# szy4017/DeepSense6G_TII

Hardware: AMD Instinct MI355X
Metric: training samples/sec (5-frame seq, bs=12 per GPU) (higher is better)
Workload: dtype f32; 1 GPU; BASELINE configs[2]: full camera+LiDAR+radar+GPS fusion, 5x(3+1+2)x256x256 + 2x2 GPS per sample, bs=12 per GPU, sigmoid focal loss, AdamW, train-mode BN, dropout 0.1; global_batch=12, seq_len=5, parallelism=dp1, ema=False, launch=eager, optimizer=AdamW after backward

## Files before the change

### deepsense6g_tii_amd/csrc/attention.hip

```cpp
#include "common.h"

int g_ds6g_attn_percu = 0;
int g_ds6g_attn_handover = 1;
int g_ds6g_attn_merged_sum = 1;
thread_local int g_attn_bwd_slab_sums = 0;
int g_ds6g_attn_fused128 = 1;

#ifdef DS6G_ATTN_CLOCKS
__device__ unsigned long long g_attn_clk[16];
extern "C" int ds6g_attn_clocks_read(unsigned long long* out16, int reset) {
    if (hipMemcpyFromSymbol(out16, HIP_SYMBOL(g_attn_clk), sizeof(unsigned long long) * 16) != hipSuccess) return -1;
    if (reset) {
        unsigned long long z[16] = {};
        if (hipMemcpyToSymbol(HIP_SYMBOL(g_attn_clk), z, sizeof(z)) != hipSuccess) return -1;
    }
    return 0;
}
#define ATTN_CLK_DECL() unsigned long long clk_t_ = 0; const bool clk_on_ = blockIdx.x == 0 && blockIdx.y == 0 && blockIdx.z == 0 && threadIdx.x == 0;
#define ATTN_CLK_START() do { __builtin_amdgcn_sched_barrier(0); clk_t_ = __builtin_readcyclecounter(); } while (0)
#define ATTN_CLK(ph) do { __builtin_amdgcn_sched_barrier(0); const unsigned long long n_ = __builtin_readcyclecounter(); \
        if (clk_on_) g_attn_clk[ph] += n_ - clk_t_; clk_t_ = n_; } while (0)
#else
#define ATTN_CLK_DECL()
#define ATTN_CLK_START()
#define ATTN_CLK(ph)
#endif

namespace {

struct AttnParams {
    const float* q;
    const float* k;
    const float* v;
    float* o;
    float* lse;
    float* ml;
    const float* d_o;
    float* delta;
    float* dq;
    float* dk;
    float* dv;
    int T, nh, B;
    int ld;
    int ldq;
    int ldd;
    int splits, tiles_per_split;
    size_t slab;
    unsigned bytes;
    unsigned bytes_q;
    float scale;
    uint32_t thr;
    float dscale;
    uint64_t seed;
    uint64_t seed_off;
    const uint64_t* salt;
    float* hs;
    float* hp;
    int nkg;
    int out16;
// ... 778 lines not shown
                ds_out[g * 64] = key_ok ? f32x4{dp[4 * g], dp[4 * g + 1], dp[4 * g + 2], dp[4 * g + 3]} : f32x4{0.f, 0.f, 0.f, 0.f};
            }
            if (PART == 2) {
                f32x4* p_out = reinterpret_cast<f32x4*>(p.hp + tile);
#pragma unroll
                for (int g = 0; g < 4; ++g)
                    p_out[g * 64] = key_ok ? f32x4{s[4 * g], s[4 * g + 1], s[4 * g + 2], s[4 * g + 3]} : f32x4{0.f, 0.f, 0.f, 0.f};
            }
        }
        __builtin_amdgcn_sched_barrier(0);
        ATTN_CLK(4);
        if (DO_DV) mma_dims<HD, BF>(dv, Oc, s, dtab);
        __builtin_amdgcn_sched_barrier(0);
        ATTN_CLK(5);
        if (DO_DK) mma_dims<HD, BF>(dk, Qc, dp, dtab);
        __builtin_amdgcn_sched_barrier(0);
        ATTN_CLK(6);
        if (HAND) asm volatile("s_waitcnt vmcnt(%0)" ::"n"((BF >= 4 ? 2 : 4) + (PART == 2 ? 4 : 0)) : "memory");
        else asm volatile("s_waitcnt vmcnt(0)" ::: "memory");
        ATTN_CLK(7);
        __syncthreads();
        ATTN_CLK(8);
#ifdef DS6G_ATTN_CLOCKS
        if (clk_on_) g_attn_clk[15] += 1;
#endif
    };

    if (t_begin < t_end) {
        q_ld.issue(Xa0, t_begin * 32, wave);
        do_ld.issue(Xb0, t_begin * 32, wave);
        stats(t_begin, 0);
    }
    asm volatile("s_waitcnt vmcnt(0)" ::: "memory");
    __syncthreads();
    for (int qt = t_begin; qt < t_end; qt += 2) {
        step(Xa0, Xb0, Xa1, Xb1, qt, 0, qt + 1 < t_end);
        if (qt + 1 < t_end) step(Xa1, Xb1, Xa0, Xb0, qt + 1, 1, qt + 2 < t_end);
    }
    if (p.splits == 1 && p.out16) {
        if (DO_DK) store_rows16<HD, BF>(dk, reinterpret_cast<typename AttnT16<BF>::T*>(p.dk) + head_offd, p.ldd, key, T, half, 1.0f);
        if (DO_DV) store_rows16<HD, BF>(dv, reinterpret_cast<typename AttnT16<BF>::T*>(p.dv) + head_offd, p.ldd, key, T, half, 1.0f);
    } else if (p.splits == 1) {
        if (DO_DK) store_rows<HD, BF>(dk, p.dk + head_offd, p.ldd, key, T, half, 1.0f);
        if (DO_DV) store_rows<HD, BF>(dv, p.dv + head_offd, p.ldd, key, T, half, 1.0f);
    } else {
        if (DO_DK) store_rows<HD, BF>(dk, p.dk + (size_t)split * p.slab + head_off, p.ld, key, T, half, 1.0f);
        if (DO_DV) store_rows<HD, BF>(dv, p.dv + (size_t)split * p.slab + head_off, p.ld, key, T, half, 1.0f);
    }
}

__global__ __launch_bounds__(256) void attn_delta_kernel(const float* __restrict__ o, const float* __restrict__ d_o,
                                                         float* __restrict__ delta, int B, int T, int nh, int hd, int ld,
                                                         int o16) {
    const long i = (long)blockIdx.x * blockDim.x + threadIdx.x;
    if (i >= (long)B * T * nh) return;
    const int h = (int)(i % nh);
    const long row = i / nh;
    const float* a = o + row * ld + h * hd;
    const float* g = d_o + row * ld + h * hd;
    float acc = 0.f;
    if (o16 == 6) {
        const _Float16* a16 = reinterpret_cast<const _Float16*>(o) + row * ld + h * hd;
        const _Float16* g16 = reinterpret_cast<const _Float16*>(d_o) + row * ld + h * hd;
        for (int d = 0; d < hd; d += 4) {
            const f32x4 x = ld4(a16 + d), y = ld4(g16 + d);
            acc += x[0] * y[0] + x[1] * y[1] + x[2] * y[2] + x[3] * y[3];
        }
    } else if (o16 == 3) {
        typedef __bf16 bf16x4_ __attribute__((ext_vector_type(4)));
        const __bf16* a16 = reinterpret_cast<const __bf16*>(o) + row * ld + h * hd;
        const __bf16* g16 = reinterpret_cast<const __bf16*>(d_o) + row * ld + h * hd;
        for (int d = 0; d < hd; d += 4) {
            const bf16x4_ x = *reinterpret_cast<const bf16x4_*>(a16 + d), y = *reinterpret_cast<const bf16x4_*>(g16 + d);
            acc += (float)x[0] * (float)y[0] + (float)x[1] * (float)y[1] + (float)x[2] * (float)y[2] + (float)x[3] * (float)y[3];
        }
    } else if (o16) {
        typedef __bf16 bf16x4_ __attribute__((ext_vector_type(4)));
        const __bf16* a16 = reinterpret_cast<const __bf16*>(o) + row * ld + h * hd;
        for (int d = 0; d < hd; d += 4) {
            const bf16x4_ x = *reinterpret_cast<const bf16x4_*>(a16 + d);
            const f32x4 y = *reinterpret_cast<const f32x4*>(g + d);
            acc += (float)x[0] * y[0] + (float)x[1] * y[1] + (float)x[2] * y[2] + (float)x[3] * y[3];
        }
    } else
    for (int d = 0; d < hd; d += 4) {
        const f32x4 x = *reinterpret_cast<const f32x4*>(a + d), y = *reinterpret_cast<const f32x4*>(g + d);
        acc += x[0] * y[0] + x[1] * y[1] + x[2] * y[2] + x[3] * y[3];
    }
    const int b = (int)(row / T), t = (int)(row % T);
    delta[((long)b * nh + h) * T + t] = acc;
}

template <int HD, int BF>
__global__ __launch_bounds__(256, 2) void attn_bwd_dq2_kernel(const AttnParams p) {
    __shared__ __attribute__((aligned(16))) float Xa0[32 * HD];
    __shared__ __attribute__((aligned(16))) float Xa1[32 * HD];
    __shared__ float Tr[4][32 * 33];
    ATTN_GEOM();
    const int q_row = bx_ * 128 + wave * 32 + l31;
    const int qt = bx_ * 4 + wave;
    const TileLoader<HD, BF> k_ld(p.k, (long)b * T * p.ldq, T, p.ldq, h * HD, wave, lane);
    f32x16 dq[NB];
#pragma unroll
    for (int blk = 0; blk < NB; ++blk)
#pragma unroll
        for (int r = 0; r < 16; ++r) dq[blk][r] = 0.f;
    const float* tiles = p.hs + (((size_t)(b * p.nh + h) * p.nkg + qt) * p.nkg) * 1024 + lane * 4;
    const bool have = qt < ntiles;
    float f[16], fn[16];
    auto fetch = [&](float* dst, int kt) {
        if (BF >= 4) {
            typedef typename AttnT16<BF>::T T16;
            typedef typename H16<T16>::x8 h8;
            const T16* t16 = reinterpret_cast<const T16*>(p.hs) + ((((size_t)(b * p.nh + h) * p.nkg + qt) * p.nkg) + kt) * 1024 + lane * 8;
#pragma unroll
            for (int g = 0; g < 2; ++g) {
                h8 v;
                if (have) v = *reinterpret_cast<const h8*>(t16 + g * 512);
#pragma unroll
                for (int e = 0; e < 8; ++e) dst[8 * g + e] = have ? (float)v[e] : 0.f;
            }
            return;
        }
#pragma unroll
        for (int g = 0; g < 4; ++g) {
            const f32x4 v = have ? *reinterpret_cast<const f32x4*>(tiles + (size_t)kt * 1024 + g * 256) : f32x4{0.f, 0.f, 0.f, 0.f};
            dst[4 * g] = v[0]; dst[4 * g + 1] = v[1]; dst[4 * g + 2] = v[2]; dst[4 * g + 3] = v[3];
        }
    };
    float* tw = Tr[wave];
    auto step = [&](const float* Kcp, const float* Kn, int kt, bool more) {
        if (more) {
            k_ld.issue(Kn, (kt + 1) * 32, wave);
            fetch(fn, kt + 1);
        }
        const unsigned Kc = opaque_tile(Kcp);
#pragma unroll
        for (int r = 0; r < 16; ++r) tw[krow16(r, half) * 33 + l31] = f[r];
        __builtin_amdgcn_wave_barrier();
        f32x16 s;
#pragma unroll
        for (int r = 0; r < 16; ++r) s[r] = tw[l31 * 33 + krow16(r, half)];
        __builtin_amdgcn_wave_barrier();
// ... 263 lines not shown
}

AttnParams attn_params(const float* q, const float* k, const float* v, int in16, float* lse, int out16, int B, int T, int nh, int hd,
                       int ld_qkv, int ld, int ld_out, float drop_p, uint64_t seed, uint64_t seed_off) {
    AttnParams p{};
    p.q = q; p.k = k; p.v = v; p.lse = lse; p.T = T; p.nh = nh; p.B = B; p.ld = ld; p.ldq = ld_qkv; p.ldd = ld_out;
    p.in16 = in16; p.out16 = out16;
    const size_t esz = in16 ? 2 : 4;
    p.slab = (size_t)B * T * ld; p.bytes = (unsigned)(p.slab * esz);
    p.bytes_q = (unsigned)((((size_t)B * T - 1) * ld_qkv + nh * hd) * esz);
    p.scale = 1.0f / sqrtf((float)hd);
    ds6g_attn_drop_params(drop_p, &p.thr, &p.dscale); p.seed = seed; p.seed_off = seed_off; p.salt = g_ds6g_salt;
    p.nkg = cdiv(T, 128) * 4;
    return p;
}

int attention_run(bool backward, const AttnParams& c, int hd, void* ws, size_t ws_bytes, void* stream) {
    const AttnKnobs kn = attn_knobs();
    const AttnShape s(c.in16 ? DS6G_ATTN_KIND_H16 : (c.out16 ? DS6G_ATTN_KIND_OUT16 : DS6G_ATTN_KIND_F32), c.B, c.T, c.nh, hd, c.ld);
    ds6g_attn_plan plan;
    int rc = DS6G_OK;
    if (backward) rc = plan_bwd(s, ws ? ws_bytes : 0, kn, &plan);
    else plan_fwd(s, ws ? ws_bytes : 0, kn, &plan);
    DS6G_CHECK_WS(rc != DS6G_ERR_WORKSPACE);
    DS6G_CHECK_ARG(rc == DS6G_OK);
    if (backward) g_attn_bwd_slab_sums = plan.slab_sums;

    static float* AttnParams::* const field[DS6G_ATTN_T_COUNT] = {&AttnParams::o, &AttnParams::ml, &AttnParams::dq, &AttnParams::dk,
                                                                   &AttnParams::dv, &AttnParams::delta, &AttnParams::hs, &AttnParams::hp};
    hipStream_t st = (hipStream_t)stream;
    AttnParams p = c;
    const int bf = c.in16 ? 3 + c.in16 : kn.bf16;
    const int cols4 = c.nh * hd / 4;
    const long n4 = (long)c.B * c.T * cols4;
    for (int i = 0; i < plan.nsteps; ++i) {
        const ds6g_attn_step& step = plan.steps[i];
        const ds6g_attn_out* o = step.out;
        float *at[3] = {}, *mine[3] = {};
        for (int j = 0; j < step.nout; ++j) { at[j] = (float*)((char*)ws + o[j].off); mine[j] = c.*field[o[j].tensor]; }
        if (step.splits) {
            p.splits = step.splits; p.tiles_per_split = step.tiles_per_split;
            for (int j = 0; j < step.nout; ++j) p.*field[o[j].tensor] = o[j].slabs ? at[j] : mine[j];
        }
        const dim3 grid(cdiv(c.T, 128), c.nh * step.splits, c.B);
        switch (step.family) {
            case DS6G_ATTN_FWD: rc = launch<DS6G_ATTN_FWD>(bf, p, hd, grid, st); break;
            case DS6G_ATTN_DQ_RECOMPUTE: rc = launch<DS6G_ATTN_DQ_RECOMPUTE>(bf, p, hd, grid, st); break;
            case DS6G_ATTN_DKV_RECOMPUTE: rc = launch<DS6G_ATTN_DKV_RECOMPUTE>(bf, p, hd, grid, st); break;
            case DS6G_ATTN_DKV_HANDOVER: rc = launch<DS6G_ATTN_DKV_HANDOVER>(bf, p, hd, grid, st); break;
            case DS6G_ATTN_DKV_FUSED128: rc = launch<DS6G_ATTN_DKV_FUSED128>(bf, p, hd, grid, st); break;
            case DS6G_ATTN_DK_TWO_PASS: rc = launch<DS6G_ATTN_DK_TWO_PASS>(bf, p, hd, grid, st); break;
            case DS6G_ATTN_DV_FROM_P: rc = launch<DS6G_ATTN_DV_FROM_P>(bf, p, hd, grid, st); break;
            case DS6G_ATTN_DQ_FROM_DS: rc = launch<DS6G_ATTN_DQ_FROM_DS>(bf, p, hd, grid, st); break;
            case DS6G_ATTN_DELTA:
                hipLaunchKernelGGL(attn_delta_kernel, dim3(cdiv((long)c.B * c.T * c.nh, 256)), dim3(256), 0, st, c.o, c.d_o, c.delta,
                                   c.B, c.T, c.nh, hd, c.ld, c.o16 | (c.in16 << 1));
                break;
            case DS6G_ATTN_FWD_MERGE:
                hipLaunchKernelGGL(attn_fwd_merge_kernel, dim3(cdiv(n4, 256)), dim3(256), 0, st, at[0], at[1], c.o, c.lse, c.B, c.T,
                                   c.nh, hd, c.ld, o[0].slabs, c.slab, c.out16);
                break;
            case DS6G_ATTN_SLAB_SUM:
                hipLaunchKernelGGL(slab_sum_kernel, dim3(cdiv(n4, 256), step.nout), dim3(256), 0, st, at[0], mine[0], at[1], mine[1],
                                   n4, cols4, c.ld, c.ldd, o[0].slabs, c.slab, c.out16, at[2], mine[2], o[2].slabs);
                break;
        }
        if (rc) return rc;
        DS6G_LAUNCH_CHECK();
    }
    return DS6G_OK;
}

}

extern "C" {

size_t ds6g_attention_workspace_bytes(int B, int T, int nh, int hd, int ld) {
    return AttnShape(DS6G_ATTN_KIND_F32, B, T, nh, hd, ld).full_workspace();
}

int ds6g_attention_plan(int backward, int kind, int B, int T, int nh, int hd, int ld, size_t ws_bytes, ds6g_attn_plan* plan) {
    DS6G_CHECK_ARG(plan && kind >= DS6G_ATTN_KIND_F32 && kind <= DS6G_ATTN_KIND_H16 && B > 0 && T > 0 && nh > 0);
    DS6G_CHECK_ARG((hd == 16 || hd == 32 || hd == 64 || hd == 128) && ld % 4 == 0 && ld >= nh * hd);
    DS6G_CHECK_ARG((size_t)B * T * ld * sizeof(float) < OOB_OFF);
    const AttnShape s(kind, B, T, nh, hd, ld);
    if (backward) return plan_bwd(s, ws_bytes, attn_knobs(), plan);
    plan_fwd(s, ws_bytes, attn_knobs(), plan);
    return DS6G_OK;
}

static int attention_fwd_impl(const float* q, const float* k, const float* v, int in16, float* o, int out16, float* lse, int B, int T,
                              int nh, int hd, int ld_qkv, int ld, float drop_p, uint64_t seed, uint64_t seed_off, void* ws,
                              size_t ws_bytes, void* stream) {
    DS6G_ENTER();
    DS6G_CHECK_ARG(q && k && v && o && lse && B > 0 && T > 0 && ld % 4 == 0 && ld >= nh * hd);
    DS6G_CHECK_ARG(ld_qkv % 4 == 0 && ld_qkv >= nh * hd && (size_t)B * T * ld_qkv * sizeof(float) < OOB_OFF);
    DS6G_CHECK_ARG(drop_p >= 0.f && drop_p < 1.f);
    DS6G_CHECK_ARG((size_t)B * T * ld * sizeof(float) < OOB_OFF);
    AttnParams c = attn_params(q, k, v, in16, lse, out16, B, T, nh, hd, ld_qkv, ld, ld, drop_p, seed, seed_off);
    c.o = o;
    return attention_run(false, c, hd, ws, ws_bytes, stream);
}

int ds6g_attention_fwd(const float* q, const float* k, const float* v, float* o, float* lse, int B, int T, int nh,
                       int hd, int ld_qkv, int ld, float drop_p, uint64_t seed, uint64_t seed_off, void* ws,
                       size_t ws_bytes, void* stream) {
    return attention_fwd_impl(q, k, v, 0, o, 0, lse, B, T, nh, hd, ld_qkv, ld, drop_p, seed, seed_off, ws, ws_bytes, stream);
}
int ds6g_attention_fwd_bf16out(const float* q, const float* k, const float* v, void* o, float* lse, int B, int T, int nh,
                               int hd, int ld_qkv, int ld, float drop_p, uint64_t seed, uint64_t seed_off, void* ws,
// ... 57 lines not shown
```

### deepsense6g_tii_amd/csrc/igemm.hip

```cpp
#include "common.h"
#include "gemm_plan.h"
#include <type_traits>
#include <vector>

extern int g_ds6g_attn_fused128;
extern int g_ds6g_attn_merged_sum;
extern int g_ds6g_attn_percu;
extern int g_ds6g_attn_handover;
extern int g_wino_kb64;

#ifndef IGEMM_STAGES_FD
#define IGEMM_STAGES_FD 3
#endif
#ifndef IGEMM_STAGES_W
#define IGEMM_STAGES_W 2
#endif

GCLK_STORAGE(g_igemm_clk, g_igemm_wg, ds6g_igemm_clocks_read)

namespace {

enum { MODE_FWD = 0, MODE_DGRAD = 1, MODE_WGRAD = 2 };

__device__ __forceinline__ unsigned opaque_u32(unsigned x) {
    asm volatile("" : "+v"(x));
    return x;
}

struct IgemmParams {
    const float* a_src;
    const float* b_src;
    float* out;
    int N, H, W, C;
    int Ho, Wo, K;
    int R, S, stride, pad;
    int Mg, Ng, Kg;
    const float* bias;
    const float* residual;
    const float* mask_src;
    int relu;
    int accumulate;
    uint32_t drop_thr;
    float drop_scale;
    uint64_t seed;
    uint64_t seed_off;
    const uint64_t* salt;
    int k_per_split;
    size_t split_stride;
    int tiles_n;
    int nclass;
    double prof_flops;
    int wg_rows;
    int is_linear;
    int want_colsum;
    int xcd_splits;
    int h0, hstep, Hs, w0, wstep, Ws, r0, rstep, nr, s0, sstep, ns;
    unsigned a_bytes, b_bytes;
    int dbg;
};


// ... 789 lines not shown
                           dim3(256), 0, st, p);
}

int run_igemm(const IgemmParams& p, const GemmPlan& pl, float* dw, float* dbias, int accumulate, hipStream_t st) {
    void* rec = ds6g_prof_open(pl.variant, p.prof_flops > 0 ? p.prof_flops : 2.0 * p.Mg * p.Ng * p.Kg, st);
    const int code = ((pl.tile * 2 + pl.epilogue) * 3 + (pl.bk == 32 ? 2 : pl.walk)) * 4 + pl.operand_mode;
    const auto codes = std::make_integer_sequence<int, 3 * 2 * 3 * 4>{};
    if (pl.mode == MODE_FWD) gemm_dispatch(code, [&](auto c) { launch_igemm<MODE_FWD, decltype(c)::value>(p, pl, st); }, codes);
    else if (pl.mode == MODE_DGRAD) gemm_dispatch(code, [&](auto c) { launch_igemm<MODE_DGRAD, decltype(c)::value>(p, pl, st); }, codes);
    else gemm_dispatch(code, [&](auto c) { launch_igemm<MODE_WGRAD, decltype(c)::value>(p, pl, st); }, codes);
    ds6g_prof_close(rec, st);
    g_last_variant = pl.variant;
    DS6G_LAUNCH_CHECK();
    if (!pl.reduce) return DS6G_OK;
    return ds6g_internal_splitk_reduce(p.out, dw, (long)pl.Mg * pl.Ng / 4, dbias, pl.want_colsum ? pl.Mg / 4 : 0, pl.splits,
                                       pl.slab_elems, accumulate, accumulate, st);
}

constexpr int F32 = DS6G_GEMM_F32;

}

extern "C" {

int ds6g_last_igemm_variant(void) { return g_last_variant; }

int ds6g_profile_begin(int max_records) {
    if (max_records <= 0) return DS6G_ERR_ARG;
    if (!g_prof) g_prof = new std::vector<ProfRec>();
    for (auto& r : *g_prof) { (void)hipEventDestroy(r.e0); (void)hipEventDestroy(r.e1); }
    g_prof->clear();
    g_prof->reserve((size_t)max_records);
    g_prof_cap = (size_t)max_records;
    return DS6G_OK;
}

int ds6g_profile_end(int* variants, double* flops, float* ms, int cap) {
    if (!g_prof) return 0;
    int n = 0;
    for (auto& r : *g_prof) {
        (void)hipEventSynchronize(r.e1);
        float t = 0.f;
        (void)hipEventElapsedTime(&t, r.e0, r.e1);
        if (n < cap && variants && flops && ms) { variants[n] = r.variant; flops[n] = r.flops; ms[n] = t; ++n; }
        (void)hipEventDestroy(r.e0);
        (void)hipEventDestroy(r.e1);
    }
    g_prof->clear();
    g_prof_cap = 0;
    return n;
}

int ds6g_set_debug_flags(int flags) {
    g_knobs.dbg = flags & 0xbf;
    g_ds6g_attn_handover = (flags & 0x01000000) ? 0 : 1;
    g_ds6g_attn_fused128 = (flags & 0x04000000) ? 0 : 1;
    g_ds6g_attn_merged_sum = (flags & 0x08000000) ? 0 : 1;
    g_ds6g_attn_percu = (flags >> 20) & 0xf;
    g_wino_kb64 = (flags & 0x02000000) ? 1 : 0;
    g_knobs.bf16_bk32 = (flags & 0x10000000) ? 0 : 1;
    g_knobs.f32_bk32 = (flags & 0x20000000) ? 1 : ((flags & 0x40000000) ? 0 : 2);
    g_knobs.wgrad_tile = (flags & 0x40) ? 2 : 1;
    if ((flags >> 8) & 0xfff) g_knobs.min_blocks = (flags >> 8) & 0xfff;
    return 0;
}

int ds6g_gemm_plan(int family, int op, int N, int H, int W, int C, int K, int R, int S, int stride, int pad, int flags,
                   size_t ws_bytes, struct ds6g_gemm_plan* plan) {
    const GemmProblem q = {family, op, N, H, W, C, K, R, S, stride, pad, (flags & DS6G_GEMM_EPILOGUE) != 0,
                           (flags & DS6G_GEMM_OUT16) != 0, (flags & DS6G_GEMM_ACCUMULATE) != 0, (flags & DS6G_GEMM_DBIAS) != 0, ws_bytes};
    return gemm_plan(q, family == DS6G_GEMM_H16 ? ds6g_internal_bgemm_knobs() : igemm_knobs(), plan);
}

int ds6g_conv2d_fwd(const float* x, const float* w, float* y, int N, int H, int W, int C, int K, int R,
                    int S, int stride, int pad, void* stream) {
    DS6G_ENTER();
    DS6G_CHECK_ARG(x && w && y);
    const GemmProblem q = {F32, DS6G_GEMM_CONV_FWD, N, H, W, C, K, R, S, stride, pad, 0, 0, 0, 0, 0};
    GemmPlan pl; IgemmParams p;
    if (const int rc = plan_params(q, pl, p)) return rc;
    p.a_src = x; p.b_src = w; p.out = y;
    return run_igemm(p, pl, nullptr, nullptr, 0, (hipStream_t)stream);
}

int ds6g_conv2d_dgrad(const float* dy, const float* w, float* dx, int N, int H, int W, int C, int K, int R,
                      int S, int stride, int pad, int accumulate, void* stream) {
    DS6G_ENTER();
    DS6G_CHECK_ARG(dy && w && dx);
    const GemmProblem q = {F32, DS6G_GEMM_CONV_DGRAD, N, H, W, C, K, R, S, stride, pad, 0, 0, accumulate, 0, 0};
    GemmPlan pl; IgemmParams p;
    if (const int rc = plan_params(q, pl, p)) return rc;
    p.a_src = dy; p.b_src = w; p.out = dx;
    return run_igemm(p, pl, nullptr, nullptr, 0, (hipStream_t)stream);
}

int ds6g_conv2d_wgrad(const float* x, const float* dy, float* dw, int N, int H, int W, int C, int K, int R,
                      int S, int stride, int pad, int accumulate, float* ws, size_t ws_bytes, void* stream) {
    DS6G_ENTER();
    DS6G_CHECK_ARG(x && dy && dw);
    const GemmProblem q = {F32, DS6G_GEMM_CONV_WGRAD, N, H, W, C, K, R, S, stride, pad, 0, 0, accumulate, 0, ws_bytes};
    GemmPlan pl; IgemmParams p;
    if (const int rc = plan_params(q, pl, p)) return rc;
    DS6G_CHECK_ARG(ws || !pl.reduce);
    p.a_src = dy; p.b_src = x; p.out = pl.reduce ? ws : dw;
    return run_igemm(p, pl, dw, nullptr, accumulate, (hipStream_t)stream);
}
// ... 53 lines not shown
```

### deepsense6g_tii_amd/csrc/norm.hip

```cpp
#include "common.h"

namespace {

constexpr int BN_ROWS_PER_THREAD = 16;
constexpr int BNF_COLS = 2;
constexpr int BNF_GROUPS = 128;

__device__ __forceinline__ void bnf_reduce2(double& a, double& b, double (*red)[4][BNF_COLS]) {
#pragma unroll
    for (int o = BNF_COLS; o < 64; o <<= 1) {
        a += __shfl_xor(a, o, 64);
        b += __shfl_xor(b, o, 64);
    }
    const int lane = threadIdx.x & 63, wave = threadIdx.x >> 6;
    if (lane < BNF_COLS) {
        red[0][wave][lane] = a;
        red[1][wave][lane] = b;
    }
    __syncthreads();
    if (threadIdx.x < BNF_COLS) {
        a = red[0][0][threadIdx.x] + red[0][1][threadIdx.x] + red[0][2][threadIdx.x] + red[0][3][threadIdx.x];
        b = red[1][0][threadIdx.x] + red[1][1][threadIdx.x] + red[1][2][threadIdx.x] + red[1][3][threadIdx.x];
    }
}

template <int MODE, typename TX, typename TA>
__global__ __launch_bounds__(256) void bn_reduce_kernel(const TX* __restrict__ x, const TA* __restrict__ dy,
                                                        const TA* __restrict__ y_mask,
                                                        const float* __restrict__ mean,
                                                        const float* __restrict__ invstd, long M, int C,
                                                        int rows_per_block, double* __restrict__ partial,
                                                        const float* __restrict__ mg, const float* __restrict__ mb,
                                                        const PoolGrad pg) {
    extern __shared__ __attribute__((aligned(16))) double red[];
    const int cg = C >> 2;
    const int colg = threadIdx.x % cg;
    const int rowlane = threadIdx.x / cg;
    const int rowlanes = 256 / cg;
    const long r0 = (long)blockIdx.x * rows_per_block;
    const long r1 = min(M, r0 + rows_per_block);
    f32x4 s1 = {0.f, 0.f, 0.f, 0.f}, s2 = {0.f, 0.f, 0.f, 0.f};
    f32x4 mu = {0.f, 0.f, 0.f, 0.f}, is = {1.f, 1.f, 1.f, 1.f};
    f32x4 gam = {1.f, 1.f, 1.f, 1.f}, bet = {0.f, 0.f, 0.f, 0.f};
    if (MODE == 1) {
        mu = *reinterpret_cast<const f32x4*>(mean + colg * 4);
        is = *reinterpret_cast<const f32x4*>(invstd + colg * 4);
        if (mg) {
            gam = *reinterpret_cast<const f32x4*>(mg + colg * 4);
            bet = *reinterpret_cast<const f32x4*>(mb + colg * 4);
        }
    }
    for (long r = r0 + rowlane; r < r1; r += rowlanes) {
        const size_t o = (size_t)r * C + colg * 4;
        const f32x4 xv = ld4(x + o);
        if (MODE == 0) {
            s1 += xv;
            s2 += xv * xv;
        } else {
            f32x4 g = pg.dp ? pooled_grad(pg, r, colg * 4, C) : ld4(dy + o);
            if (y_mask || mg) {
                const f32x4 yv = mg ? bn_affine(xv, mu, is, gam, bet) : ld4(y_mask + o);
#pragma unroll
                for (int j = 0; j < 4; ++j) g[j] = yv[j] > 0.f ? g[j] : 0.f;
            }
            s1 += g;
            s2 += g * ((xv - mu) * is);
        }
    }
    double* mine = red + ((size_t)rowlane * 2) * C + colg * 4;
#pragma unroll
    for (int j = 0; j < 4; ++j) {
        mine[j] = (double)s1[j];
        mine[C + j] = (double)s2[j];
    }
    __syncthreads();
    for (int i = threadIdx.x; i < 2 * C; i += 256) {
        double acc = 0.0;
        for (int rl = 0; rl < rowlanes; ++rl) acc += red[(size_t)rl * 2 * C + i];
        partial[(size_t)blockIdx.x * 2 * C + i] = acc;
    }
}

__global__ __launch_bounds__(256) void bn_stats_finalize_kernel(const double* __restrict__ partial, int nblk, long M,
                                                                int C, float eps, float momentum,
                                                                float* __restrict__ mean, float* __restrict__ invstd,
                                                                float* __restrict__ running_mean,
                                                                float* __restrict__ running_var) {
    __shared__ double red[2][4][BNF_COLS];
    const int cl = threadIdx.x & (BNF_COLS - 1), g = threadIdx.x / BNF_COLS;
    const int c = blockIdx.x * BNF_COLS + cl;
    double s = 0.0, q = 0.0;
    if (c < C)
        for (int b = g; b < nblk; b += BNF_GROUPS) {
            s += partial[(size_t)b * 2 * C + c];
            q += partial[(size_t)b * 2 * C + C + c];
        }
    bnf_reduce2(s, q, red);
    if (g != 0 || c >= C) return;
    const double mu = s / (double)M;
    double var = q / (double)M - mu * mu;
    if (var < 0.0) var = 0.0;
    mean[c] = (float)mu;
    invstd[c] = (float)(1.0 / sqrt(var + (double)eps));
    if (running_mean) {
        const double unbiased = M > 1 ? var * ((double)M / (double)(M - 1)) : var;
        running_mean[c] = (float)((1.0 - momentum) * (double)running_mean[c] + momentum * mu);
        running_var[c] = (float)((1.0 - momentum) * (double)running_var[c] + momentum * unbiased);
    }
}

__global__ void bn_eval_prepare_kernel(const float* __restrict__ running_mean, const float* __restrict__ running_var,
                                       int C, float eps, float* __restrict__ mean, float* __restrict__ invstd) {
    const int c = blockIdx.x * blockDim.x + threadIdx.x;
    if (c >= C) return;
    mean[c] = running_mean[c];
    invstd[c] = 1.0f / sqrtf(running_var[c] + eps);
// ... 11 lines not shown
        const int c4 = (int)(i % cg) * 4;
        const f32x4 mu = *reinterpret_cast<const f32x4*>(mean + c4);
        const f32x4 is = *reinterpret_cast<const f32x4*>(invstd + c4);
        const f32x4 g = *reinterpret_cast<const f32x4*>(gamma + c4);
        const f32x4 b = *reinterpret_cast<const f32x4*>(beta + c4);
        f32x4 v = ld4(x + i * 4);
        v = bn_affine(v, mu, is, g, b);
        if (residual) v += ld4(residual + i * 4);
        if (relu) {
#pragma unroll
            for (int j = 0; j < 4; ++j) v[j] = fmaxf(v[j], 0.f);
        }
        st4(y + i * 4, v);
    }
}

__global__ __launch_bounds__(256) void bn_bwd_finalize_kernel(const double* __restrict__ partial, int nblk, long M,
                                                              int C, const float* __restrict__ gamma,
                                                              const float* __restrict__ invstd,
                                                              float* __restrict__ dgamma, float* __restrict__ dbeta,
                                                              float* __restrict__ coef, int accumulate) {
    __shared__ double red[2][4][BNF_COLS];
    const int cl = threadIdx.x & (BNF_COLS - 1), g = threadIdx.x / BNF_COLS;
    const int c = blockIdx.x * BNF_COLS + cl;
    double s1 = 0.0, s2 = 0.0;
    if (c < C)
        for (int b = g; b < nblk; b += BNF_GROUPS) {
            s1 += partial[(size_t)b * 2 * C + c];
            s2 += partial[(size_t)b * 2 * C + C + c];
        }
    bnf_reduce2(s1, s2, red);
    if (g != 0 || c >= C) return;
    if (accumulate) {
        dgamma[c] += (float)s2;
        dbeta[c] += (float)s1;
    } else {
        dgamma[c] = (float)s2;
        dbeta[c] = (float)s1;
    }
    coef[c] = gamma[c] * invstd[c];
    coef[C + c] = (float)(s1 / (double)M);
    coef[2 * C + c] = (float)(s2 / (double)M);
}

template <typename TX, typename TA>
__global__ __launch_bounds__(256) void bn_bwd_apply_kernel(const TA* __restrict__ dy,
                                                           const TA* __restrict__ y_mask,
                                                           const TX* __restrict__ x,
                                                           const float* __restrict__ mean,
                                                           const float* __restrict__ invstd,
                                                           const float* __restrict__ coef, TX* __restrict__ dx,
                                                           TA* __restrict__ dres, long total4, int C,
                                                           const float* __restrict__ mg, const float* __restrict__ mb,
                                                           const PoolGrad pg) {
    const int cg = C >> 2;
    for (long i = (long)blockIdx.x * blockDim.x + threadIdx.x; i < total4; i += (long)gridDim.x * blockDim.x) {
        const int c4 = (int)(i % cg) * 4;
        const f32x4 mu = *reinterpret_cast<const f32x4*>(mean + c4);
        const f32x4 is = *reinterpret_cast<const f32x4*>(invstd + c4);
        const f32x4 a = *reinterpret_cast<const f32x4*>(coef + c4);
        const f32x4 b = *reinterpret_cast<const f32x4*>(coef + C + c4);
        const f32x4 cc = *reinterpret_cast<const f32x4*>(coef + 2 * C + c4);
        f32x4 g = pg.dp ? pooled_grad(pg, i / cg, c4, C) : ld4(dy + i * 4);
        const f32x4 xv = ld4(x + i * 4);
        if (y_mask || mg) {
            const f32x4 yv = mg ? bn_affine(xv, mu, is, *reinterpret_cast<const f32x4*>(mg + c4),
                                            *reinterpret_cast<const f32x4*>(mb + c4))
                                : ld4(y_mask + i * 4);
#pragma unroll
            for (int j = 0; j < 4; ++j) g[j] = yv[j] > 0.f ? g[j] : 0.f;
        }
        const f32x4 xh = (xv - mu) * is;
        if (dres) st4(dres + i * 4, g);
        st4(dx + i * 4, a * (g - b - xh * cc));
    }
}

int bn_geometry(long M, int C, int* rows_per_block, int* nblk) {
    const int cg = C / 4;
    if (C % 4 != 0 || cg > 256 || 256 % cg != 0) return DS6G_ERR_ARG;
    *rows_per_block = BN_ROWS_PER_THREAD * (256 / cg);
    *nblk = cdiv(M, *rows_per_block);
    return DS6G_OK;
}

template <int C>
struct LnRow {
    static constexpr bool VEC = C >= 256;
    static constexpr int NV = VEC ? C / 256 : C / 64;
    static constexpr int NE = VEC ? 4 * NV : NV;
    __device__ static void load(float* v, const float* row, int lane) {
        if (VEC) {
#pragma unroll
            for (int j = 0; j < NV; ++j) {
                const f32x4 t = *reinterpret_cast<const f32x4*>(row + 4 * lane + 256 * j);
                v[4 * j] = t[0]; v[4 * j + 1] = t[1]; v[4 * j + 2] = t[2]; v[4 * j + 3] = t[3];
            }
        } else {
#pragma unroll
            for (int j = 0; j < NV; ++j) v[j] = row[lane + 64 * j];
        }
    }
    __device__ static void store(const float* v, float* row, int lane) {
        if (VEC) {
#pragma unroll
            for (int j = 0; j < NV; ++j)
                *reinterpret_cast<f32x4*>(row + 4 * lane + 256 * j) = f32x4{v[4 * j], v[4 * j + 1], v[4 * j + 2], v[4 * j + 3]};
        } else {
#pragma unroll
            for (int j = 0; j < NV; ++j) row[lane + 64 * j] = v[j];
        }
    }
    __device__ static int col(int e, int lane) { return VEC ? 4 * lane + 256 * (e >> 2) + (e & 3) : lane + 64 * e; }
    template <typename T16>
    __device__ static void load(float* v, const T16* row, int lane) {
        typedef typename H16<T16>::x4 h4;
        if (VEC) {
#pragma unroll
            for (int j = 0; j < NV; ++j) {
                const h4 t = *reinterpret_cast<const h4*>(row + 4 * lane + 256 * j);
                v[4 * j] = (float)t[0]; v[4 * j + 1] = (float)t[1]; v[4 * j + 2] = (float)t[2]; v[4 * j + 3] = (float)t[3];
            }
        } else {
#pragma unroll
            for (int j = 0; j < NV; ++j) v[j] = (float)row[lane + 64 * j];
        }
// ... 168 lines not shown
    const int rowlanes = 256 / cols_per_pass;
    const int rowlane = threadIdx.x / cols_per_pass;
    const long r0 = (long)blockIdx.x * rows_per_block;
    const long r1 = min(M, r0 + rows_per_block);
    for (int cbase = 0; cbase < cg; cbase += cols_per_pass) {
        const int colg = cbase + threadIdx.x % cols_per_pass;
        f32x4 s = {0.f, 0.f, 0.f, 0.f};
        if (colg < cg)
            for (long r = r0 + rowlane; r < r1; r += rowlanes) s += *reinterpret_cast<const f32x4*>(x + (size_t)r * C + colg * 4);
        if (colg < cg) *reinterpret_cast<f32x4*>(redf + (size_t)rowlane * C + colg * 4) = s;
    }
    __syncthreads();
    for (int c = threadIdx.x; c < C; c += 256) {
        float acc = 0.f;
        for (int rl = 0; rl < rowlanes; ++rl) acc += redf[(size_t)rl * C + c];
        partial[(size_t)blockIdx.x * C + c] = acc;
    }
}

template <typename TW>
__global__ __launch_bounds__(256) void bn_fold_kernel(const float* __restrict__ w, const float* __restrict__ gamma,
                                                      const float* __restrict__ beta, const float* __restrict__ mean,
                                                      const float* __restrict__ var, float eps, TW* __restrict__ w_out,
                                                      float* __restrict__ bias_out, int K, int taps, int cin, int cpad) {
    const long i = (long)blockIdx.x * blockDim.x + threadIdx.x;
    const long per_o = (long)taps * cpad;
    if (i >= (long)K * per_o) return;
    const int o = (int)(i / per_o);
    const int rem = (int)(i - (long)o * per_o);
    const int tap = rem / cpad, c = rem - tap * cpad;
    const float scale = gamma[o] / sqrtf(var[o] + eps);
    float v = c < cin ? w[((long)o * taps + tap) * cin + c] * scale : 0.f;
    if constexpr (sizeof(TW) == 2) asm volatile("" : "+v"(v));
    w_out[i] = (TW)v;
    if (rem == 0) bias_out[o] = beta[o] - mean[o] * scale;
}

}

extern "C" size_t ds6g_layernorm_bwd_workspace_bytes(int M, int C);
extern "C" size_t ds6g_bn_workspace_bytes(long M, int C);

template <typename TX>
static int bn_stats_run(const TX* x, long M, int C, float eps, float momentum, float* mean, float* invstd,
                        float* running_mean, float* running_var, void* ws, size_t ws_bytes, void* stream) {
    int rpb, nblk;
    DS6G_CHECK_ARG(x && mean && invstd && ws && M > 0);
    DS6G_CHECK_ARG(bn_geometry(M, C, &rpb, &nblk) == DS6G_OK);
    DS6G_CHECK_WS(ws_bytes >= ds6g_bn_workspace_bytes(M, C));
    double* partial = (double*)ws;
    const size_t lds = (size_t)(256 / (C / 4)) * 2 * C * sizeof(double);
    hipLaunchKernelGGL((bn_reduce_kernel<0, TX, TX>), dim3(nblk), dim3(256), lds, (hipStream_t)stream, x, (const TX*)nullptr,
                       (const TX*)nullptr, (const float*)nullptr, (const float*)nullptr, M, C, rpb, partial,
                       (const float*)nullptr, (const float*)nullptr, PoolGrad{});
    DS6G_LAUNCH_CHECK();
    hipLaunchKernelGGL(bn_stats_finalize_kernel, dim3(cdiv(C, BNF_COLS)), dim3(256), 0, (hipStream_t)stream, partial, nblk,
                       M, C, eps, momentum, mean, invstd, running_mean, running_var);
    DS6G_LAUNCH_CHECK();
    return DS6G_OK;
}

template <typename TA>
static int bn_apply_run(const TA* x, const float* mean, const float* invstd, const float* gamma, const float* beta,
                        const TA* residual, TA* y, long M, int C, int relu, void* stream) {
    DS6G_CHECK_ARG(x && mean && invstd && gamma && beta && y && C % 4 == 0);
    const long total4 = M * C / 4;
    const int grid = (int)min((long)8192, (total4 + 255) / 256);
    hipLaunchKernelGGL((bn_apply_kernel<TA>), dim3(grid), dim3(256), 0, (hipStream_t)stream, x, mean, invstd, gamma, beta,
                       residual, y, total4, C, relu);
    DS6G_LAUNCH_CHECK();
    return DS6G_OK;
}

template <typename TX, typename TA>
static int bn_bwd_run(const TA* dy, const PoolGrad pg, const TA* y_mask, const TX* x, const float* mean,
                      const float* invstd, const float* gamma, const float* relu_beta, TX* dx, float* dgamma,
                      float* dbeta, TA* dres, long M, int C, int accumulate_param_grads, void* ws, size_t ws_bytes,
                      void* stream) {
    const float* mg = relu_beta ? gamma : nullptr;
    int rpb, nblk;
    DS6G_CHECK_ARG(bn_geometry(M, C, &rpb, &nblk) == DS6G_OK);
    DS6G_CHECK_WS(ws_bytes >= ds6g_bn_workspace_bytes(M, C));
    double* partial = (double*)ws;
    float* coef = (float*)((char*)ws + (size_t)nblk * 2 * C * sizeof(double));
    const size_t lds = (size_t)(256 / (C / 4)) * 2 * C * sizeof(double);
    hipLaunchKernelGGL((bn_reduce_kernel<1, TX, TA>), dim3(nblk), dim3(256), lds, (hipStream_t)stream, x, dy, y_mask, mean,
                       invstd, M, C, rpb, partial, mg, relu_beta, pg);
    DS6G_LAUNCH_CHECK();
    hipLaunchKernelGGL(bn_bwd_finalize_kernel, dim3(cdiv(C, BNF_COLS)), dim3(256), 0, (hipStream_t)stream, partial, nblk, M,
                       C, gamma, invstd, dgamma, dbeta, coef, accumulate_param_grads);
    DS6G_LAUNCH_CHECK();
    const long total4 = M * C / 4;
    const int grid = (int)min((long)8192, (total4 + 255) / 256);
    hipLaunchKernelGGL((bn_bwd_apply_kernel<TX, TA>), dim3(grid), dim3(256), 0, (hipStream_t)stream, dy, y_mask, x, mean,
                       invstd, coef, dx, dres, total4, C, mg, relu_beta, pg);
    DS6G_LAUNCH_CHECK();
    return DS6G_OK;
}

template <typename TY>
static int ln_fwd_launch(const float* x, const float* gamma, const float* beta, TY* y, float* mean, float* rstd, int M, int C,
                         float eps, hipStream_t st) {
    dim3 grid(cdiv(M, 4)), block(256);
    switch (C / 64) {
        case 1: hipLaunchKernelGGL((ln_fwd_kernel<64, TY>), grid, block, 0, st, x, gamma, beta, y, mean, rstd, M, eps); break;
        case 2: hipLaunchKernelGGL((ln_fwd_kernel<128, TY>), grid, block, 0, st, x, gamma, beta, y, mean, rstd, M, eps); break;
        case 4: hipLaunchKernelGGL((ln_fwd_kernel<256, TY>), grid, block, 0, st, x, gamma, beta, y, mean, rstd, M, eps); break;
        case 8: hipLaunchKernelGGL((ln_fwd_kernel<512, TY>), grid, block, 0, st, x, gamma, beta, y, mean, rstd, M, eps); break;
        default: DS6G_CHECK_ARG(!"LayerNorm width must be 64/128/256/512");
    }
    DS6G_LAUNCH_CHECK();
    return DS6G_OK;
}

template <typename TDY, typename TDD>
static int ln_bwd_launch(const TDY* dy, const float* x, const float* mean, const float* rstd, const float* gamma,
                         const float* add, float* dx, float* dgamma, float* dbeta, int M, int C, int accumulate_param_grads,
                         TDD* dx_drop, float drop_p, uint64_t seed, uint64_t seed_off, void* ws, size_t ws_bytes,
                         hipStream_t st, bool defer = false) {
    DS6G_CHECK_ARG(dy && x && mean && rstd && gamma && dx && (defer || (dgamma && dbeta)) && ws && M > 0);
    DS6G_CHECK_ARG(drop_p >= 0.f && drop_p < 1.f);
    const uint32_t thr = ds6g_drop_threshold(drop_p);
    const float dscale = 1.f / (1.f - drop_p);
    DS6G_CHECK_ARG(C % 64 == 0 && C <= 512);
    DS6G_CHECK_WS(ws_bytes >= ds6g_layernorm_bwd_workspace_bytes(M, C));
    const int nblk = cdiv(M, LN_BWD_ROWS);
    float* partial = (float*)ws;
    dim3 grid(nblk), block(256);
    switch (C / 64) {
        case 1: hipLaunchKernelGGL((ln_bwd_kernel<64, TDY, TDD>), grid, block, 0, st, dy, x, mean, rstd, gamma, add, dx, partial, M, dx_drop, thr, dscale, seed, seed_off, g_ds6g_salt); break;
        case 2: hipLaunchKernelGGL((ln_bwd_kernel<128, TDY, TDD>), grid, block, 0, st, dy, x, mean, rstd, gamma, add, dx, partial, M, dx_drop, thr, dscale, seed, seed_off, g_ds6g_salt); break;
        case 4: hipLaunchKernelGGL((ln_bwd_kernel<256, TDY, TDD>), grid, block, 0, st, dy, x, mean, rstd, gamma, add, dx, partial, M, dx_drop, thr, dscale, seed, seed_off, g_ds6g_salt); break;
        case 8: hipLaunchKernelGGL((ln_bwd_kernel<512, TDY, TDD>), grid, block, 0, st, dy, x, mean, rstd, gamma, add, dx, partial, M, dx_drop, thr, dscale, seed, seed_off, g_ds6g_salt); break;
        default: DS6G_CHECK_ARG(!"LayerNorm width must be 64/128/256/512");
    }
    DS6G_LAUNCH_CHECK();
    if (defer) return DS6G_OK;
    hipLaunchKernelGGL(col_finalize_kernel, dim3(cdiv(2 * C, 4)), dim3(256), 0, st, partial, nblk, 2 * C, dgamma,
                       dbeta, C, accumulate_param_grads);
    DS6G_LAUNCH_CHECK();
    return DS6G_OK;
}

int ds6g_internal_bn_stats_finalize(const double* partial, int nblk, long M, int C, float eps, float momentum, float* mean,
                                    float* invstd, float* running_mean, float* running_var, hipStream_t st) {
    hipLaunchKernelGGL(bn_stats_finalize_kernel, dim3(cdiv(C, BNF_COLS)), dim3(256), 0, st, partial, nblk, M, C, eps,
                       momentum, mean, invstd, running_mean, running_var);
    DS6G_LAUNCH_CHECK();
// ... 280 lines not shown
```

Before: 187.7 samples/s.

## Coalesce attention delta reduction and reuse masked BN grad from reduce pass

Adds a streaming attention-delta kernel in which threads load contiguous quads of o and dO, with coalesced accesses, and write partial dot products to LDS. A second loop sums each head's terms, replacing the one-thread-per-row strided loop. Separately, the BN backward reduce pass now stores the ReLU-masked gradient into dres, so the apply pass reads it back instead of re-reading dy and y_mask. Both paths are on by default with debug flags to revert, and fp contraction is disabled so the delta arithmetic stays consistent between the two kernels.

```diff
diff --git a/deepsense6g_tii_amd/csrc/attention.hip b/deepsense6g_tii_amd/csrc/attention.hip
--- a/deepsense6g_tii_amd/csrc/attention.hip
+++ b/deepsense6g_tii_amd/csrc/attention.hip
@@ -5,6 +5,7 @@
 int g_ds6g_attn_merged_sum = 1;
 thread_local int g_attn_bwd_slab_sums = 0;
 int g_ds6g_attn_fused128 = 1;
+int g_ds6g_attn_delta_serial = 0;
 
 #ifdef DS6G_ATTN_CLOCKS
 __device__ unsigned long long g_attn_clk[16];
@@ -889,6 +890,7 @@
 __global__ __launch_bounds__(256) void attn_delta_kernel(const float* __restrict__ o, const float* __restrict__ d_o,
                                                          float* __restrict__ delta, int B, int T, int nh, int hd, int ld,
                                                          int o16) {
+#pragma clang fp contract(off)
     const long i = (long)blockIdx.x * blockDim.x + threadIdx.x;
     if (i >= (long)B * T * nh) return;
     const int h = (int)(i % nh);
@@ -926,6 +928,62 @@
     }
     const int b = (int)(row / T), t = (int)(row % T);
     delta[((long)b * nh + h) * T + t] = acc;
+}
+
+constexpr int DELTA_QUADS = 1024;
+
+__device__ __forceinline__ float delta_quad(const f32x4 x, const f32x4 y) {
+#pragma clang fp contract(off)
+    return x[0] * y[0] + x[1] * y[1] + x[2] * y[2] + x[3] * y[3];
+}
+
+template <typename TO, typename TG>
+__global__ __launch_bounds__(256) void attn_delta_stream_kernel(const TO* __restrict__ o, const TG* __restrict__ d_o,
+                                                                float* __restrict__ delta, long rows, int T, int nh, int hd,
+                                                                int ld, int rows_per_block) {
+    extern __shared__ float terms[];
+    const int qh = hd >> 2, qr = nh * qh;
+    const long row0 = (long)blockIdx.x * rows_per_block;
+    const int nrow = (int)min((long)rows_per_block, rows - row0);
+    const int nq = nrow * qr;
+    for (int q0 = threadIdx.x; q0 < nq; q0 += DELTA_QUADS) {
+        f32x4 x[4], y[4];
+#pragma unroll
+        for (int u = 0; u < 4; ++u) {
+            const int q = q0 + u * 256;
+            if (q < nq) {
+                const int r = q / qr, cq = q - r * qr;
+                const size_t off = (size_t)(row0 + r) * ld + cq * 4;
+                x[u] = ld4(o + off);
+                y[u] = ld4(d_o + off);
+            }
+        }
+#pragma unroll
+        for (int u = 0; u < 4; ++u) {
+            const int q = q0 + u * 256;
+            if (q < nq) {
+                const int r = q / qr, cq = q - r * qr;
+                terms[r * nh * (qh + 1) + cq + cq / qh] = delta_quad(x[u], y[u]);
+            }
+        }
+    }
+    __syncthreads();
+    for (int c = threadIdx.x; c < nrow * nh; c += 256) {
+        const float* t = terms + c * (qh + 1);
+        float acc = 0.f;
+        for (int k = 0; k < qh; ++k) acc += t[k];
+        const int r = c / nh, h = c - r * nh;
+        const long row = row0 + r;
+        delta[((row / T) * nh + h) * T + row % T] = acc;
+    }
+}
+
+int delta_rows_per_block(long rows, int nh, int hd) {
+    const int qr = nh * (hd / 4);
+    int quads = DELTA_QUADS;
+    while (quads > 256 && cdiv(rows, quads / qr > 0 ? quads / qr : 1) < 512) quads /= 2;
+    const int rpb = quads / qr > 0 ? quads / qr : 1;
+    return (size_t)rpb * nh * (hd / 4 + 1) * sizeof(float) <= 48 * 1024 ? rpb : 0;
 }
 
 template <int HD, int BF>
@@ -1295,10 +1353,29 @@
             case DS6G_ATTN_DK_TWO_PASS: rc = launch<DS6G_ATTN_DK_TWO_PASS>(bf, p, hd, grid, st); break;
             case DS6G_ATTN_DV_FROM_P: rc = launch<DS6G_ATTN_DV_FROM_P>(bf, p, hd, grid, st); break;
             case DS6G_ATTN_DQ_FROM_DS: rc = launch<DS6G_ATTN_DQ_FROM_DS>(bf, p, hd, grid, st); break;
-            case DS6G_ATTN_DELTA:
-                hipLaunchKernelGGL(attn_delta_kernel, dim3(cdiv((long)c.B * c.T * c.nh, 256)), dim3(256), 0, st, c.o, c.d_o, c.delta,
-                                   c.B, c.T, c.nh, hd, c.ld, c.o16 | (c.in16 << 1));
+            case DS6G_ATTN_DELTA: {
+                const long rows = (long)c.B * c.T;
+                const int o16 = c.o16 | (c.in16 << 1);
+                const int rpb = g_ds6g_attn_delta_serial ? 0 : delta_rows_per_block(rows, c.nh, hd);
+                if (!rpb) {
+                    hipLaunchKernelGGL(attn_delta_kernel, dim3(cdiv(rows * c.nh, 256)), dim3(256), 0, st, c.o, c.d_o, c.delta,
+                                       c.B, c.T, c.nh, hd, c.ld, o16);
+                    break;
+                }
+                const dim3 dgrid(cdiv(rows, rpb));
+                const size_t lds = (size_t)rpb * c.nh * (hd / 4 + 1) * sizeof(float);
+                const __bf16 *ob = (const __bf16*)c.o, *gb = (const __bf16*)c.d_o;
+                const _Float16 *oh = (const _Float16*)c.o, *gh = (const _Float16*)c.d_o;
+                if (o16 == 6)
+                    hipLaunchKernelGGL((attn_delta_stream_kernel<_Float16, _Float16>), dgrid, dim3(256), lds, st, oh, gh, c.delta, rows, c.T, c.nh, hd, c.ld, rpb);
+                else if (o16 == 3)
+                    hipLaunchKernelGGL((attn_delta_stream_kernel<__bf16, __bf16>), dgrid, dim3(256), lds, st, ob, gb, c.delta, rows, c.T, c.nh, hd, c.ld, rpb);
+                else if (o16)
+                    hipLaunchKernelGGL((attn_delta_stream_kernel<__bf16, float>), dgrid, dim3(256), lds, st, ob, c.d_o, c.delta, rows, c.T, c.nh, hd, c.ld, rpb);
+                else
+                    hipLaunchKernelGGL((attn_delta_stream_kernel<float, float>), dgrid, dim3(256), lds, st, (const float*)c.o, c.d_o, c.delta, rows, c.T, c.nh, hd, c.ld, rpb);
                 break;
+            }
             case DS6G_ATTN_FWD_MERGE:
                 hipLaunchKernelGGL(attn_fwd_merge_kernel, dim3(cdiv(n4, 256)), dim3(256), 0, st, at[0], at[1], c.o, c.lse, c.B, c.T,
                                    c.nh, hd, c.ld, o[0].slabs, c.slab, c.out16);
diff --git a/deepsense6g_tii_amd/csrc/igemm.hip b/deepsense6g_tii_amd/csrc/igemm.hip
--- a/deepsense6g_tii_amd/csrc/igemm.hip
+++ b/deepsense6g_tii_amd/csrc/igemm.hip
@@ -7,6 +7,8 @@
 extern int g_ds6g_attn_merged_sum;
 extern int g_ds6g_attn_percu;
 extern int g_ds6g_attn_handover;
+extern int g_ds6g_attn_delta_serial;
+extern int g_ds6g_bn_dres_twice;
 extern int g_wino_kb64;
 
 #ifndef IGEMM_STAGES_FD
@@ -902,6 +904,10 @@
 }
 
 int ds6g_set_debug_flags(int flags) {
+    const int helper = (flags & (int)0x80000000) ? flags & 3 : 0;
+    if (flags & (int)0x80000000) flags &= ~0x3f;
+    g_ds6g_attn_delta_serial = helper & 1;
+    g_ds6g_bn_dres_twice = (helper >> 1) & 1;
     g_knobs.dbg = flags & 0xbf;
     g_ds6g_attn_handover = (flags & 0x01000000) ? 0 : 1;
     g_ds6g_attn_fused128 = (flags & 0x04000000) ? 0 : 1;
diff --git a/deepsense6g_tii_amd/csrc/norm.hip b/deepsense6g_tii_amd/csrc/norm.hip
--- a/deepsense6g_tii_amd/csrc/norm.hip
+++ b/deepsense6g_tii_amd/csrc/norm.hip
@@ -1,4 +1,6 @@
 #include "common.h"
+
+int g_ds6g_bn_dres_twice = 0;
 
 namespace {
 
@@ -31,7 +33,7 @@
                                                         const float* __restrict__ invstd, long M, int C,
                                                         int rows_per_block, double* __restrict__ partial,
                                                         const float* __restrict__ mg, const float* __restrict__ mb,
-                                                        const PoolGrad pg) {
+                                                        const PoolGrad pg, TA* __restrict__ dres) {
     extern __shared__ __attribute__((aligned(16))) double red[];
     const int cg = C >> 2;
     const int colg = threadIdx.x % cg;
@@ -62,6 +64,7 @@
                 const f32x4 yv = mg ? bn_affine(xv, mu, is, gam, bet) : ld4(y_mask + o);
 #pragma unroll
                 for (int j = 0; j < 4; ++j) g[j] = yv[j] > 0.f ? g[j] : 0.f;
+                if (MODE == 1 && dres) st4(dres + o, g);
             }
             s1 += g;
             s2 += g * ((xv - mu) * is);
@@ -179,7 +182,7 @@
                                                            const float* __restrict__ coef, TX* __restrict__ dx,
                                                            TA* __restrict__ dres, long total4, int C,
                                                            const float* __restrict__ mg, const float* __restrict__ mb,
-                                                           const PoolGrad pg) {
+                                                           const PoolGrad pg, int g_in_dres) {
     const int cg = C >> 2;
     for (long i = (long)blockIdx.x * blockDim.x + threadIdx.x; i < total4; i += (long)gridDim.x * blockDim.x) {
         const int c4 = (int)(i % cg) * 4;
@@ -188,9 +191,9 @@
         const f32x4 a = *reinterpret_cast<const f32x4*>(coef + c4);
         const f32x4 b = *reinterpret_cast<const f32x4*>(coef + C + c4);
         const f32x4 cc = *reinterpret_cast<const f32x4*>(coef + 2 * C + c4);
-        f32x4 g = pg.dp ? pooled_grad(pg, i / cg, c4, C) : ld4(dy + i * 4);
+        f32x4 g = g_in_dres ? ld4(dres + i * 4) : pg.dp ? pooled_grad(pg, i / cg, c4, C) : ld4(dy + i * 4);
         const f32x4 xv = ld4(x + i * 4);
-        if (y_mask || mg) {
+        if (!g_in_dres && (y_mask || mg)) {
             const f32x4 yv = mg ? bn_affine(xv, mu, is, *reinterpret_cast<const f32x4*>(mg + c4),
                                             *reinterpret_cast<const f32x4*>(mb + c4))
                                 : ld4(y_mask + i * 4);
@@ -198,7 +201,7 @@
             for (int j = 0; j < 4; ++j) g[j] = yv[j] > 0.f ? g[j] : 0.f;
         }
         const f32x4 xh = (xv - mu) * is;
-        if (dres) st4(dres + i * 4, g);
+        if (dres && !g_in_dres) st4(dres + i * 4, g);
         st4(dx + i * 4, a * (g - b - xh * cc));
     }
 }
@@ -473,7 +476,7 @@
     const size_t lds = (size_t)(256 / (C / 4)) * 2 * C * sizeof(double);
     hipLaunchKernelGGL((bn_reduce_kernel<0, TX, TX>), dim3(nblk), dim3(256), lds, (hipStream_t)stream, x, (const TX*)nullptr,
                        (const TX*)nullptr, (const float*)nullptr, (const float*)nullptr, M, C, rpb, partial,
-                       (const float*)nullptr, (const float*)nullptr, PoolGrad{});
+                       (const float*)nullptr, (const float*)nullptr, PoolGrad{}, (TX*)nullptr);
     DS6G_LAUNCH_CHECK();
     hipLaunchKernelGGL(bn_stats_finalize_kernel, dim3(cdiv(C, BNF_COLS)), dim3(256), 0, (hipStream_t)stream, partial, nblk,
                        M, C, eps, momentum, mean, invstd, running_mean, running_var);
@@ -505,8 +508,9 @@
     double* partial = (double*)ws;
     float* coef = (float*)((char*)ws + (size_t)nblk * 2 * C * sizeof(double));
     const size_t lds = (size_t)(256 / (C / 4)) * 2 * C * sizeof(double);
+    const int g_in_dres = y_mask && dres && !pg.dp && !g_ds6g_bn_dres_twice;
     hipLaunchKernelGGL((bn_reduce_kernel<1, TX, TA>), dim3(nblk), dim3(256), lds, (hipStream_t)stream, x, dy, y_mask, mean,
-                       invstd, M, C, rpb, partial, mg, relu_beta, pg);
+                       invstd, M, C, rpb, partial, mg, relu_beta, pg, g_in_dres ? dres : (TA*)nullptr);
     DS6G_LAUNCH_CHECK();
     hipLaunchKernelGGL(bn_bwd_finalize_kernel, dim3(cdiv(C, BNF_COLS)), dim3(256), 0, (hipStream_t)stream, partial, nblk, M,
                        C, gamma, invstd, dgamma, dbeta, coef, accumulate_param_grads);
@@ -514,7 +518,7 @@
     const long total4 = M * C / 4;
     const int grid = (int)min((long)8192, (total4 + 255) / 256);
     hipLaunchKernelGGL((bn_bwd_apply_kernel<TX, TA>), dim3(grid), dim3(256), 0, (hipStream_t)stream, dy, y_mask, x, mean,
-                       invstd, coef, dx, dres, total4, C, mg, relu_beta, pg);
+                       invstd, coef, dx, dres, total4, C, mg, relu_beta, pg, g_in_dres);
     DS6G_LAUNCH_CHECK();
     return DS6G_OK;
 }
```

After: 187.6 samples/s, median of 2. No clear change (-0.1%).
